# CliffKai/BridgeLang

Hardware: AMD Instinct MI355X
Metric: action-seqs/sec (7-DoF, 224px) openvla-7b bf16 (higher is better)
Workload: dtype bf16; 1 GPU; openvla-7b bf16 inference (BASELINE configs[1]): batch 16 synthetic 224px frames + 32-token prompts per GPU, predict_action = vision towers + projector + Llama prefill S=288 + 6 cached decode steps, greedy; 7 batches in flight: per step one batch is submitted (vision+prefill) while decode iteration g of the batch submitted g steps earlier, g = 1..6, runs as ONE merged 96-row pass over the weights ; batch_per_gpu=16, prompt_len=32, seq_len=288, replicas=1, hip_graph=True, pipeline_depth=7

## Files before the change

### bridgelang_amd/_lib.py

```python
from __future__ import annotations

import ctypes as C
import os
from pathlib import Path

_HERE = Path(__file__).resolve().parent
LIB_PATH = _HERE / "libbridgelang_hip.so"

BL_OK, BL_E_SHAPE, BL_E_ALIGN, BL_E_LAUNCH, BL_E_ARG = 0, -1, -2, -3, -4
_ERR = {BL_E_SHAPE: "BL_E_SHAPE (unsupported shape)", BL_E_ALIGN: "BL_E_ALIGN (alignment)",
        BL_E_LAUNCH: "BL_E_LAUNCH (HIP launch failed)", BL_E_ARG: "BL_E_ARG (null pointer / bad enum)"}

EPI_NONE, EPI_BIAS, EPI_BIAS_GELU, EPI_BIAS_RES, EPI_RES, EPI_SWIGLU, EPI_F32, EPI_F32_BF16R = range(8)
EPI_SWIGLU_KEEP, EPI_BIAS_GELU_KEEP, EPI_SWIGLU_BWD, EPI_GELU_BWD = range(8, 12)


class GemmDesc(C.Structure):
    _fields_ = [
        ("A", C.c_void_p), ("lda", C.c_int64),
        ("W", C.c_void_p), ("ldw", C.c_int64),
        ("C", C.c_void_p), ("ldc", C.c_int64),
        ("M", C.c_int32), ("N", C.c_int32), ("K", C.c_int32),
        ("epilogue", C.c_int32),
        ("bias", C.c_void_p),
# ... 22 lines not shown
        ("k", C.c_void_p), ("k_bs", C.c_int64), ("k_hs", C.c_int64), ("k_rs", C.c_int64),
        ("v", C.c_void_p), ("v_bs", C.c_int64), ("v_hs", C.c_int64), ("v_rs", C.c_int64),
        ("o", C.c_void_p), ("o_bs", C.c_int64), ("o_hs", C.c_int64), ("o_rs", C.c_int64),
        ("key_mask", C.c_void_p), ("mask_bs", C.c_int64),
        ("B", C.c_int32), ("H", C.c_int32), ("Sq", C.c_int32), ("Skv", C.c_int32), ("head_dim", C.c_int32),
        ("causal", C.c_int32),
        ("scale", C.c_float),
    ]


_vp, _i32, _i64, _u32, _f32 = C.c_void_p, C.c_int32, C.c_int64, C.c_uint32, C.c_float

SIGNATURES = {
    "bl_abi_version": (C.c_int, []),
    "bl_build_arch": (C.c_char_p, []),
    "bl_fill_synth_bf16": (C.c_int, [_vp, _i64, _u32, _f32, _f32, _vp]),
    "bl_fill_synth_bf16_2d": (C.c_int, [_vp, _i64, _i64, _i64, _u32, _f32, _f32, _vp]),
    "bl_pack_weight_bf16": (C.c_int, [_vp, _i64, _i64, _i64, _vp, _vp]),
    "bl_gemm_fp8": (C.c_int, [C.POINTER(GemmDesc), _vp, _vp, _vp]),
    "bl_quantize_rows_fp8": (C.c_int, [_vp, _i64, _i32, _i32, _vp, _i64, _vp, _vp]),
    "bl_colamax_bf16": (C.c_int, [_vp, _i64, _i32, _i32, _vp, _vp]),
    "bl_transpose_quantize_fp8": (C.c_int, [_vp, _i64, _i32, _i32, _vp, _vp, _i64, _i32, _vp, _vp]),
    "bl_gemm_bf16": (C.c_int, [C.POINTER(GemmDesc), _vp]),
    "bl_gemm_skinny_bf16": (C.c_int, [C.POINTER(GemmDesc), _vp]),
    "bl_gemm_skinny_rows_bf16": (C.c_int, [C.POINTER(GemmDesc), _vp]),
    "bl_gemm_tn_bf16": (C.c_int, [C.POINTER(GemmDesc), _vp]),
    "bl_rmsnorm_skinny_bf16": (C.c_int, [_vp, _i64, _vp, _vp, _i64, _i32, _i32, _f32, _vp]),
    "bl_layernorm_bf16": (C.c_int, [_vp, _i64, _vp, _vp, _vp, _i64, _i32, _i32, _f32, _vp]),
    "bl_rmsnorm_bf16": (C.c_int, [_vp, _i64, _vp, _vp, _i64, _i32, _i32, _f32, _vp]),
    "bl_attention_bf16": (C.c_int, [C.POINTER(AttnDesc), _vp]),
    "bl_attention_rope_bf16": (C.c_int, [C.POINTER(AttnDesc), _vp, _vp, _i32, _vp, _vp, _i32, _vp]),
    "bl_attention_lse_bf16": (C.c_int, [C.POINTER(AttnDesc), _vp, _vp]),
    "bl_attention_backward_bf16": (C.c_int, [C.POINTER(AttnDesc), _vp, _vp, _vp, _vp, _vp, _vp, _vp]),
    "bl_attention_decode_bf16": (C.c_int, [C.POINTER(AttnDesc), _vp]),
    "bl_attention_decode_rope_bf16": (C.c_int, [C.POINTER(AttnDesc), _vp, _vp, _i32, _vp]),
    "bl_attention_decode_rope_pos_bf16": (C.c_int, [C.POINTER(AttnDesc), _vp, _vp, _i32, _vp, _vp]),
    "bl_attention_decode_rope_grouped_bf16": (C.c_int, [C.POINTER(AttnDesc), _vp, _vp, _i32, _vp, _vp, _vp, _vp]),
    "bl_rope_kvcache_bf16": (C.c_int, [_vp, _i32, _i32, _i32, _i32, _vp, _vp, _i32, _vp, _vp, _i32, _vp]),
    "bl_embed_splice_bf16": (C.c_int, [_vp, _i32, _i32, _vp, _i32, _i32, _vp, _vp]),
    "bl_argmax_f32": (C.c_int, [_vp, _i64, _i32, _i32, _vp, _vp]),
    "bl_cross_entropy_f32": (C.c_int, [_vp, _i64, _i32, _i32, _vp, _i64, _vp, _vp, _vp]),
    "bl_cross_entropy_backward_f32": (C.c_int, [_vp, _i64, _i32, _i32, _vp, _i64, _vp, _vp, _i64, _vp]),
    "bl_rmsnorm_backward_bf16": (C.c_int, [_vp, _i64, _vp, _vp, _i64, _vp, _i64, _vp, _i64, _vp, _vp, _i64, _i32, _i32, _f32, _vp]),
    "bl_layernorm_backward_bf16": (C.c_int, [_vp, _i64, _vp, _vp, _i64, _vp, _i64, _vp, _i64, _vp, _vp, _vp, _i64, _i32, _i32, _f32, _vp]),
    "bl_colsum_bf16": (C.c_int, [_vp, _i64, _i32, _i32, _vp, _vp, _i64, _vp]),
    "bl_swiglu_bf16": (C.c_int, [_vp, _i64, _vp, _i64, _i64, _i32, _vp]),
# ... 63 lines not shown
```

### bridgelang_amd/csrc/gemm_bf16.hip

```cpp
#include "gemm_common.h"
#include <stdlib.h>

namespace bl_gemm_bf16_impl {
using namespace blgemm;

constexpr int BK = 64;
constexpr int ROW_BYTES = 128;
constexpr int GROUP_M = 4;

__device__ __forceinline__ void lin_to_tile(const GemmArgs& p, int lin, int& tm, int& tn) {
  const int width = GROUP_M * p.tiles_n, grp = lin / width, first = grp * GROUP_M;
  const int gsz = min(p.tiles_m - first, GROUP_M), rem = lin - grp * width;
  tm = first + rem % gsz;
  tn = rem / gsz;
}

__device__ __forceinline__ void tile_coords(const GemmArgs& p, int& tm, int& tn) {
  const int nwg = gridDim.x;
  const int orig = blockIdx.x, xcd = orig & 7, q = nwg >> 3, r = nwg & 7;
  const int lin = (xcd < r ? xcd * (q + 1) : r * (q + 1) + (xcd - r) * q) + (orig >> 3);
  const int width = GROUP_M * p.tiles_n, grp = lin / width, first = grp * GROUP_M;
  const int gsz = min(p.tiles_m - first, GROUP_M), rem = lin - grp * width;
  tm = first + rem % gsz;
  tn = rem / gsz;
// ... 210 lines not shown
    BL_KSTEP(0, 1, kt);
    BL_KSTEP(1, 0, kt + 1);
  }
  if (nk & 1) BL_KSTEP(0, 1, nk - 1);
#undef BL_KSTEP
#undef BL_READ
  asm volatile("s_waitcnt vmcnt(0)" ::: "memory");
#undef BL_PIECE
  if (sliced) {
    float* slab = p.slab + (long)blockIdx.y * p.M * p.N;
#pragma unroll
    for (int i = 0; i < NT; ++i)
#pragma unroll
      for (int j = 0; j < MT; ++j) {
        const int m = m0 + wm * TM + j * 16 + l15, n = n0 + wn * TN + i * 16 + lg * 4;
        if (m < p.M && n < p.N) *(f32x4_t*)(slab + (long)m * p.N + n) = acc[i][j];
      }
    return;
  }
  int ncol[NT];
#pragma unroll
  for (int i = 0; i < NT; ++i) ncol[i] = n0 + wn * TN + i * 16 + lg * 4;
  epilogue_tile<EPI, NT, MT>(p, m0 + wm * TM + l15, ncol, m0 + BM, n0 + BN, acc);
#endif
}

template <int EPI>
__global__ __launch_bounds__(256) void gemm128_splitk_reduce_kernel(GemmArgs p) {
#if defined(__HIP_DEVICE_COMPILE__)
  const int n4 = p.N >> 2;
  const long total = (long)p.M * n4;
  for (long i = (long)blockIdx.x * 256 + threadIdx.x; i < total; i += (long)gridDim.x * 256) {
    const int m = (int)(i / n4), n = (int)(i - (long)m * n4) * 4;
    f32x4_t sum = *(const f32x4_t*)(p.slab + (long)m * p.N + n);
    for (int s2 = 1; s2 < p.splitk; ++s2) sum += *(const f32x4_t*)(p.slab + ((long)s2 * p.M + m) * p.N + n);
    epilogue_store4<EPI>(p, m, n, sum);
  }
#endif
}

template <int EPI>
__global__ __launch_bounds__(256) void gemm_rows_tree_reduce_kernel(GemmArgs p) {
#if defined(__HIP_DEVICE_COMPILE__)
  const int n4 = p.N >> 2, S = p.splitk;
  const long total = (long)p.M * n4, stride = (long)p.M * p.N;
  for (long i = (long)blockIdx.x * 256 + threadIdx.x; i < total; i += (long)gridDim.x * 256) {
// ... 948 lines not shown
        lds_attr(&gemm_ring8_kernel<EPI, 64, 64, 4>, ring8_lds_bytes(64, 64)) &&
        lds_attr(&gemm_mid2_kernel<EPI, 1>, 3 * (160 * ROW_BYTES + 4096)) &&
        lds_attr(&gemm_mid2_kernel<EPI, 4>, 3 * (160 * ROW_BYTES + 4 * 4096)) &&
        lds_attr(&gemm_mid2_kernel<EPI, 2, 2>, 2 * (160 * ROW_BYTES + 2 * 4096)) &&
        mid_attr<EPI, 2, 4>() && mid_attr<EPI, 4, 4>() && mid_attr<EPI, 5, 4>() && mid_attr<EPI, 2, 1>() &&
        mid_attr<EPI, 4, 1>() && mid_attr<EPI, 5, 1>();
    return ok ? BL_OK : BL_E_LAUNCH;
  }();
  return rc;
}

template <int EPI>
void launch_slab_reduce(const GemmArgs& p, hipStream_t s) {
  const long work = (long)p.M * (p.N / 4);
  hipLaunchKernelGGL((gemm128_splitk_reduce_kernel<EPI>), dim3((int)min((work + 255) / 256, 2048L)), dim3(256), 0, s, p);
}

template <int EPI, int MB>
void launch_mid(const GemmArgs& p, hipStream_t s, bool wide, dim3 grid) {
  if (wide) hipLaunchKernelGGL((gemm_mid_kernel<EPI, MB, 4>), grid, dim3(256), (mid_lds_bytes<MB, 4>()), s, p);
  else hipLaunchKernelGGL((gemm_mid_kernel<EPI, MB, 1>), grid, dim3(256), (mid_lds_bytes<MB, 1>()), s, p);
}

template <int EPI>
int launch_gemm(const GemmArgs& a, hipStream_t s) {
  if (set_lds_attr<EPI>() != BL_OK) return BL_E_LAUNCH;
  GemmArgs p = a;
  const int bm = (p.M + 255) / 256, bn = (p.N + 255) / 256, big_tiles = bm * bn;
  const bool big = big_tiles >= 128 && p.K >= 512;
  const bool mid2_only = p.M > 320;
  if (p.M <= 640 && p.M > 32 && p.K >= 512 && !(mid2_only && (p.slab || (p.N % 32)))) {
    const int slabs64 = (p.N + 63) / 64, nkm = p.K / BK;
    bool wide = slabs64 >= 160;
    int S = 1;
    if (!wide && p.slab && slabs64 * 2 <= CUS) {
      int S2 = min(8, CUS / slabs64);
      while (S2 > 1 && (nkm / S2 < 8 || p.slab_bytes < (long)S2 * p.M * p.N * 4)) --S2;
      if (S2 > 1) { wide = true; S = S2; }
    }
    if (S == 1 && p.M > 128 && (p.N % 32) == 0) {
      const int mb = (p.M + 159) / 160;
      if (!wide)
        hipLaunchKernelGGL((gemm_mid2_kernel<EPI, 1>), dim3(p.N / 32, mb), dim3(256), 3 * (160 * ROW_BYTES + 4096), s, p);
      else if (slabs64 >= 400)
        hipLaunchKernelGGL((gemm_mid2_kernel<EPI, 4>), dim3((p.N + 127) / 128, mb), dim3(256), 3 * (160 * ROW_BYTES + 4 * 4096), s, p);
      else
        hipLaunchKernelGGL((gemm_mid2_kernel<EPI, 2, 2>), dim3((p.N + 63) / 64, mb), dim3(256), 2 * (160 * ROW_BYTES + 2 * 4096), s, p);
      BL_CHECK_LAUNCH();
      return BL_OK;
    }
    const int slabs = wide ? slabs64 : (p.N + 15) / 16;
    if (S == 1 && !wide && p.slab && slabs < CUS) {
      S = min(8, (CUS + CUS / 2 + slabs - 1) / slabs);
      while (S > 1 && (nkm / S < 8 || p.slab_bytes < (long)S * p.M * p.N * 4)) --S;
    }
    p.splitk = S;
    const dim3 grid(slabs, S);
    if (p.M <= 128) launch_mid<EPI, 2>(p, s, wide, grid);
    else if (p.M <= 256) launch_mid<EPI, 4>(p, s, wide, grid);
    else launch_mid<EPI, 5>(p, s, wide, grid);
    if (S > 1) launch_slab_reduce<EPI>(p, s);
    BL_CHECK_LAUNCH();
    return BL_OK;
  }
  if (!big && p.K >= 512) {
    const int t160 = ((p.M + 159) / 160) * ((p.N + 127) / 128);
    if (t160 <= CUS && t160 >= (3 * CUS) / 4) {
      p.tiles_m = (p.M + 159) / 160;
      p.tiles_n = (p.N + 127) / 128;
      p.tail_base = -1;
      hipLaunchKernelGGL((gemm_ring8_kernel<EPI, 160, 128, 4>), dim3(t160), dim3(512), ring8_lds_bytes(160, 128), s, p);
      BL_CHECK_LAUNCH();
      return BL_OK;
    }
  }
  if (!big) {
    p.tiles_m = (p.M + 127) / 128;
    p.tiles_n = (p.N + 127) / 128;
    const int tiles = p.tiles_m * p.tiles_n, nk128 = p.K / BK;
    int S128 = 1;
    if (p.slab && tiles <= CUS / 2) {
      S128 = min(8, CUS / tiles);
      while (S128 > 1 && (nk128 / S128 < 8 || p.slab_bytes < (long)S128 * p.M * p.N * 4)) --S128;
    }
    if (S128 > 1) {
      p.splitk = S128;
      hipLaunchKernelGGL((gemm_ring8_kernel<EPI, 128, 128, 4>), dim3(tiles, S128), dim3(512), ring8_lds_bytes(128, 128), s, p);
      launch_slab_reduce<EPI>(p, s);
    } else {
      hipLaunchKernelGGL((gemm128_kernel<EPI>), dim3(tiles), dim3(256), LDS128, s, p);
// ... 34 lines not shown
  const bool can_split = tail && S >= 2 && p.K >= 8192 && p.slab && p.slab_bytes >= (long)tail * S * 256 * 256 * 4;
  if (can_split) {
    main_tiles = big_tiles - tail;
    if (main_tiles) launch256(main_tiles);
    p.tail_base = main_tiles;
    p.splitk = S;
    launch256(tail * S);
    hipLaunchKernelGGL((gemm_splitk_reduce_kernel<EPI>), dim3(tail * 32), dim3(512), 0, s, p);
  } else {
    if (tail != 0 && tail <= 64 && main_tiles > tail) main_tiles = big_tiles - tail; else tail = 0;
    launch256(main_tiles);
    if (tail) {
      p.tail_base = main_tiles;
      if (tail <= 16)
        hipLaunchKernelGGL((gemm_ring8_kernel<EPI, 64, 64, 4>), dim3(tail * 16), dim3(512), ring8_lds_bytes(64, 64), s, p);
      else if (tail <= 32)
        hipLaunchKernelGGL((gemm_ring8_kernel<EPI, 128, 64, 4>), dim3(tail * 8), dim3(512), ring8_lds_bytes(128, 64), s, p);
      else
        hipLaunchKernelGGL((gemm_ring8_kernel<EPI, 128, 128, 4>), dim3(tail * 4), dim3(512), ring8_lds_bytes(128, 128), s, p);
    }
  }
  BL_CHECK_LAUNCH();
  return BL_OK;
}

int launch_gemm_tn(const GemmArgs& a, hipStream_t s) {
  static const int attr_rc = lds_attr(&gemm256s_kernel<BL_EPI_F32, true>, LDS256) ? BL_OK : BL_E_LAUNCH;
  if (attr_rc != BL_OK) return attr_rc;
  GemmArgs p = a;
  p.tiles_m = (p.M + 255) / 256;
  p.tiles_n = (p.N + 255) / 256;
  const int tiles = p.tiles_m * p.tiles_n, nk = (p.K + BK - 1) / BK;
  int tail = tiles > CUS ? tiles % CUS : (2 * tiles <= CUS ? tiles : 0);
  int S = tail ? CUS / tail : 1;
  if (tiles <= CUS && S > 8) S = 8;
  if (S > 16) S = 16;
  while (S > 1 && nk / S < 4) --S;
  const bool can_split = tail && S >= 2 && (nk >= 128 || tiles <= CUS) && p.slab &&
                         p.slab_bytes >= (long)tail * S * 256 * 256 * 4;
  const bool persist_ok = (nk % 2) == 0 && ((long)(p.K - 1) * p.lda + p.M) * 2 < (1L << 32) &&
                          ((long)(p.K - 1) * p.ldw + p.N) * 2 < (1L << 32);
  auto launch_main = [&](int grid) {
    if (persist_ok && grid > CUS) {
      GemmArgs pp = p;
      pp.ptiles = grid;
      hipLaunchKernelGGL((gemm256s_kernel<BL_EPI_F32, true>), dim3(CUS), dim3(512), LDS256, s, pp);
// ... 20 lines not shown
extern "C" int bl_gemm_bf16(const bl_gemm_desc* d, void* stream) {
  GemmArgs a;
  const int rc = fill_gemm_args(d, a);
  if (rc != BL_OK) return rc;
  if (d->a_norm_weight) return BL_E_ARG;
  hipStream_t s = (hipStream_t)stream;
  switch (d->epilogue) {
    case BL_EPI_NONE: return launch_gemm<BL_EPI_NONE>(a, s);
    case BL_EPI_BIAS: return launch_gemm<BL_EPI_BIAS>(a, s);
    case BL_EPI_BIAS_GELU: return launch_gemm<BL_EPI_BIAS_GELU>(a, s);
    case BL_EPI_BIAS_RES: return launch_gemm<BL_EPI_BIAS_RES>(a, s);
    case BL_EPI_RES: return launch_gemm<BL_EPI_RES>(a, s);
    case BL_EPI_SWIGLU: return launch_gemm<BL_EPI_SWIGLU>(a, s);
    case BL_EPI_F32: return launch_gemm<BL_EPI_F32>(a, s);
    case BL_EPI_F32_BF16R: return launch_gemm<BL_EPI_F32_BF16R>(a, s);
    case BL_EPI_SWIGLU_KEEP: return launch_gemm<BL_EPI_SWIGLU_KEEP>(a, s);
    case BL_EPI_BIAS_GELU_KEEP: return launch_gemm<BL_EPI_BIAS_GELU_KEEP>(a, s);
    case BL_EPI_SWIGLU_BWD: return launch_gemm<BL_EPI_SWIGLU_BWD>(a, s);
    case BL_EPI_GELU_BWD: return launch_gemm<BL_EPI_GELU_BWD>(a, s);
    default: return BL_E_ARG;
  }
}

extern "C" int bl_gemm_skinny_rows_bf16(const bl_gemm_desc* d, void* stream) {
  GemmArgs a;
  const int rc = fill_gemm_args(d, a);
  if (rc != BL_OK) return rc;
  if (d->M > 128 || (d->K % 256) || d->a_norm_weight) return BL_E_SHAPE;
  if (d->out_group) return BL_E_ARG;
  hipStream_t s = (hipStream_t)stream;
  switch (d->epilogue) {
    case BL_EPI_NONE: return launch_rows_sk<BL_EPI_NONE>(a, s);
    case BL_EPI_RES: return launch_rows_sk<BL_EPI_RES>(a, s);
    case BL_EPI_SWIGLU: return launch_rows_sk<BL_EPI_SWIGLU>(a, s);
    case BL_EPI_F32: return launch_rows_sk<BL_EPI_F32>(a, s);
    case BL_EPI_F32_BF16R: return launch_rows_sk<BL_EPI_F32_BF16R>(a, s);
    default: return BL_E_ARG;
  }
}

extern "C" int bl_gemm_tn_bf16(const bl_gemm_desc* d, void* stream) {
  if (!d || !d->A || !d->W || !d->C) return BL_E_ARG;
  if (d->epilogue != BL_EPI_F32 || d->out_group || d->a_norm_weight) return BL_E_ARG;
  if (d->M <= 0 || d->N <= 0 || d->K <= 0 || (d->M % 8) || (d->N % 8)) return BL_E_SHAPE;
  if ((d->lda % 8) || (d->ldw % 8) || (d->ldc % 4) || d->lda < d->M || d->ldw < d->N || d->ldc < d->N) return BL_E_ALIGN;
  if (!bl_aligned16(d->A) || !bl_aligned16(d->W) || (((uintptr_t)d->C) & 15)) return BL_E_ALIGN;
// ... 10 lines not shown
```

### bridgelang_amd/engine.py

```python
from __future__ import annotations

from typing import List, Optional

import torch

from . import ops
from .ops import EPI_BIAS, EPI_BIAS_GELU, EPI_BIAS_RES, EPI_F32_BF16R, EPI_NONE, EPI_RES, EPI_SWIGLU, Op
from .weights import TowerW, VLAWeights


def rope_tables(head_dim: int, max_pos: int, theta: float, device) -> tuple:
    inv = 1.0 / (theta ** (torch.arange(0, head_dim, 2, dtype=torch.int64).float() / head_dim))
    fr = torch.arange(max_pos, dtype=torch.float32)[:, None] * inv[None, :]
    return fr.cos().to(torch.bfloat16).to(device), fr.sin().to(torch.bfloat16).to(device)


def _fp8_layers(weights: VLAWeights) -> list:
    cache = weights.__dict__.get("_fp8_layers")
    if cache is None:
        cache = [{n: ops.quantize_weight_fp8(ops.unpack_weight(getattr(lw, n))) for n in ("qkv_w", "o_w", "gu_w", "down_w")}
                 for lw in weights.layers]
        weights.__dict__["_fp8_layers"] = cache
    return cache

# ... 51 lines not shown
            self.qkvd, self.actd = z(B, 3 * D), z(B, I)
        self.cos, self.sin = rope_tables(d.head_dim, d.max_pos, d.rope_theta, dev)
        self.ws = torch.empty(64 << 20, dtype=torch.uint8, device=dev) if splitk else None
        if padded:
            if d.head_dim != 128 or not ops.skinny_supported(B, D, EPI_NONE):
                raise NotImplementedError("padded generation needs head_dim 128 and a batch of at most 16")
            self.cache_mask = torch.ones(B, self.cache_len, dtype=torch.uint8, device=dev)
            self.key_mask = self.cache_mask[:, :S]
            self.last_row = torch.full((B,), S - 1, dtype=torch.int64, device=dev)
            self.rope_pos = torch.zeros(n_new, B, dtype=torch.int32, device=dev)
            self.q_last, self.x_last = z(B, 3 * D), z(B, D)
            self._rows = torch.arange(B, device=dev)
        else:
            self.key_mask = torch.ones(B, S, dtype=torch.uint8, device=dev) if use_mask else None
        self.logits_all = z(B * S, d.vocab, dtype=torch.float32) if all_rows else None
        self.fp8 = fp8
        if fp8:
            if d.llm_dim % 128 or d.llm_inter % 128:
                raise ValueError("fp8 prefill needs llm_dim and llm_inter to be multiples of 128")
            self.w8 = _fp8_layers(weights)
            self.h8, self.act8 = z(B * S, D, dtype=torch.uint8), z(B * S, I, dtype=torch.uint8)
            self.sq = z(B * S, dtype=torch.float32)

        self.dino_ops = [] if text_only else self._plan_tower(weights.dino, 0, self.vbuf[0])
        self.siglip_ops = [] if text_only else self._plan_tower(weights.siglip, d.dino.dim, self.vbuf[1])
        self.vision_ops = self.dino_ops + self.siglip_ops
        self._side = torch.cuda.Stream(device=dev) if dev.type == "cuda" else None
        if vision_only:
            self.projector_ops, self.prefill_ops, self.decode_ops = [], [], []
        else:
            self.projector_ops = [] if text_only else self._plan_projector()
            self.prefill_ops = self._plan_prefill()
            self.decode_ops = [self._plan_decode(t) for t in range(1, n_new)]
        self._graph: Optional[torch.cuda.CUDAGraph] = None

    def _g(self, *args, **kw):
        return ops.gemm(*args, workspace=self.ws, **kw)

    def _plan_tower(self, tw: TowerW, feat_col: int, vb: dict) -> List[Op]:
        t, B = tw.dims, self.B
        T, Dm, Hp, hd = t.tokens, t.dim, t.mlp_pad, t.head_dim
        M = B * T
        x = vb["x"][:M * Dm].view(M, Dm)
        h = vb["h"][:M * Dm].view(M, Dm)
        ao = vb["ao"][:M * Dm].view(M, Dm)
        qkv = vb["qkv"][:M * 3 * Dm].view(M, 3 * Dm)
        mlp = vb["mlp"][:M * Hp].view(M, Hp)
        v_col = vb["col"]
        g = lambda *a, **k: ops.gemm(*a, workspace=vb["ws"], **k)
        plan = [ops.im2col_patch14(self.pixel_values, t.chan0, v_col, run=False)]
        if tw.prefix is not None:
            plan.append(ops.write_prefix_tokens(tw.prefix, x, B, T, run=False))
        plan.append(g(v_col, tw.patch_w, x, EPI_BIAS_RES, bias=tw.patch_b, res=tw.pos, res_row_mod=256,
                             out_map=(256, T, t.n_prefix), algo_nk=(Dm, self.dims.patch_k), run=False))
        st = (T * 3 * Dm, hd, 3 * Dm)
        for i, b in enumerate(tw.blocks):
            plan.append(ops.layernorm(x, b.norm1_w, b.norm1_b, h, self.dims.ln_eps, run=False))
            plan.append(g(h, b.qkv_w, qkv, EPI_BIAS, bias=b.qkv_b, run=False))
            plan.append(ops.attention(qkv, qkv[:, Dm:], qkv[:, 2 * Dm:], ao, B=B, H=t.heads, Sq=T, Skv=T, head_dim=hd,
                                      q_strides=st, k_strides=st, v_strides=st, o_strides=(T * Dm, hd, Dm),
                                      causal=False, run=False))
            plan.append(g(ao, b.proj_w, x, EPI_BIAS_RES, bias=b.proj_b, scale=b.ls1, res=x, run=False))
            plan.append(ops.layernorm(x, b.norm2_w, b.norm2_b, h, self.dims.ln_eps, run=False))
            plan.append(g(h, b.fc1_w, mlp, EPI_BIAS_GELU, bias=b.fc1_b, algo_nk=(t.mlp, Dm), run=False))
            if i + 1 < len(tw.blocks):
                plan.append(g(mlp, b.fc2_w, x, EPI_BIAS_RES, bias=b.fc2_b, scale=b.ls2, res=x, algo_nk=(Dm, t.mlp),
                                     run=False))
            else:
                plan.append(g(mlp, b.fc2_w, self.feats[:, feat_col:feat_col + Dm], EPI_BIAS_RES, bias=b.fc2_b,
                                     scale=b.ls2, res=x, out_map=(T, 256, -t.n_prefix), algo_nk=(Dm, t.mlp), run=False))
        return plan

    def _plan_projector(self) -> List[Op]:
        w, B, S, D = self.w, self.B, self.S, self.dims.llm_dim
        return [self._g(self.feats, w.fc1_w, self.p1, EPI_BIAS_GELU, bias=w.fc1_b, run=False),
                self._g(self.p1, w.fc2_w, self.p2, EPI_BIAS_GELU, bias=w.fc2_b, run=False),
                self._g(self.p2, w.fc3_w, self.x.view(B * S, D), EPI_BIAS, bias=w.fc3_b, out_map=(256, S, 1), run=False)]

    def _plan_prefill(self, b0: int = 0, b1: Optional[int] = None) -> List[Op]:
        d, w, S = self.dims, self.w, self.S
        b1 = self.B if b1 is None else b1
        B = b1 - b0
        D, H, hd = d.llm_dim, d.llm_heads, d.head_dim
        rows = slice(b0 * S, b1 * S)
        x3 = self.x[b0:b1]
        x = x3.view(B * S, D)
        h, qkv, ao, act = self.h[rows], self.qkv[rows], self.ao[rows], self.act[rows]
        xd, hdd, aod, actd = self.xd[b0:b1], self.hd[b0:b1], self.aod[b0:b1], self.actd[b0:b1]
        key_mask = self.key_mask[b0:b1] if self.key_mask is not None else None
        plan = [ops.embed_splice(self.input_ids[b0:b1], w.embed, x3, self.n_patches, run=False)]
        self.layer_ends: List[int] = []
        cs = (H * self.cache_len * hd, self.cache_len * hd, hd)
        last_rows_only = not self.all_rows and d.llm_layers > 1
        for l, lw in enumerate(w.layers):
# ... 96 lines not shown
                plan.append(self._g(self.hd, lw.qkv_w, self.qkvd, EPI_NONE, run=False))
                plan.append(ops.rope_kvcache(self.qkvd, self.cos, self.sin, self.k_cache[l], self.v_cache[l], B=B, S=1,
                                             H=H, head_dim=hd, pos0=pos, run=False))
                plan.append(ops.attention_decode(self.qkvd, self.k_cache[l], self.v_cache[l], self.aod, B=B, H=H,
                                                 Skv=pos + 1, head_dim=hd, q_strides=(3 * D, hd, 3 * D), k_strides=cs,
                                                 v_strides=cs, o_strides=(D, hd, D), run=False))
            plan.append(self._g(self.aod, lw.o_w, self.xd, EPI_RES, res=self.xd, run=False))
            if fused:
                plan.append(self._g(self.xd, lw.gu_w, self.actd, EPI_SWIGLU, a_norm=(lw.ln2, d.rms_eps), run=False))
            else:
                plan.append(ops.rmsnorm(self.xd, lw.ln2, self.hd, d.rms_eps, run=False))
                plan.append(self._g(self.hd, lw.gu_w, self.actd, EPI_SWIGLU, run=False))
            plan.append(self._g(self.actd, lw.down_w, self.xd, EPI_RES, res=self.xd, run=False))
        plan += self._head(self.xd, t)
        return plan

    def all_ops(self) -> List[Op]:
        out = self.vision_ops + self.projector_ops + self.prefill_ops
        for step in self.decode_ops:
            out = out + step
        return out

    def run_vision(self) -> None:
        if self._side is None:
            ops.run_all(self.vision_ops)
            return
        main = torch.cuda.current_stream()
        self._side.wait_stream(main)
        with torch.cuda.stream(self._side):
            ops.run_all(self.siglip_ops)
        ops.run_all(self.dino_ops)
        main.wait_stream(self._side)

    def _run_all_stages(self) -> None:
        self.run_vision()
        ops.run_all(self.projector_ops + self.prefill_ops)
        for step in self.decode_ops:
            ops.run_all(step)

    def run_eager(self) -> None:
        self._run_all_stages()

    def capture(self) -> None:
        self.run_eager()
        torch.cuda.synchronize()
        g = torch.cuda.CUDAGraph()
# ... 47 lines not shown
```

### bridgelang_amd/ops.py

```python
from __future__ import annotations

import functools
import math

import ctypes as C
from typing import Optional, Sequence, Tuple

import torch

from . import _lib
from ._lib import (AttnDesc, GemmDesc, EPI_BIAS, EPI_BIAS_GELU, EPI_BIAS_GELU_KEEP, EPI_BIAS_RES, EPI_F32, EPI_F32_BF16R, EPI_GELU_BWD,
                   EPI_NONE, EPI_SWIGLU_BWD, EPI_SWIGLU_KEEP,
                   EPI_RES, EPI_SWIGLU)

__all__ = ["Op", "gemm", "gemm_fp8", "quantize_rows_fp8", "quantize_weight_fp8", "pack_weight", "unpack_weight", "cross_entropy", "layernorm", "rmsnorm", "rmsnorm_skinny", "skinny_rows_supported", "attention", "attention_rope", "attention_decode", "attention_decode_rope", "attention_decode_rope_grouped", "skinny_supported", "rope_kvcache", "embed_splice",
           "argmax", "im2col_patch14", "preprocess_u8", "resample_coeffs", "resize_bicubic_u8", "resize_u8", "crop_resize_bilinear_u8", "write_prefix_tokens", "fill_synth", "run_all",
           "EPI_NONE", "EPI_BIAS", "EPI_BIAS_GELU", "EPI_BIAS_RES", "EPI_RES", "EPI_SWIGLU", "EPI_F32", "EPI_F32_BF16R",
           "EPI_SWIGLU_KEEP", "EPI_BIAS_GELU_KEEP", "EPI_SWIGLU_BWD", "EPI_GELU_BWD"]


def _stream() -> int:
    return torch.cuda.current_stream().cuda_stream


def _bf16(t: torch.Tensor, what: str) -> torch.Tensor:
    if t.dtype != torch.bfloat16 or not t.is_cuda:
        raise TypeError(f"{what}: expected a CUDA/HIP bfloat16 tensor, got {t.dtype} on {t.device}")
    return t


def _rows(t: torch.Tensor, what: str) -> int:
    if t.dim() != 2 or t.stride(1) != 1:
        raise ValueError(f"{what}: expected a 2-D tensor with contiguous last dim, got shape {tuple(t.shape)} "
                         f"stride {t.stride()}")
    return t.stride(0) if t.shape[0] > 1 else max(t.stride(0), t.shape[1])


class Op:
# ... 109 lines not shown
    if use_skinny is None:
        use_skinny = skinny_supported(M, K, epilogue)
    if a_norm is not None:
        if not use_skinny:
            raise ValueError("gemm: a_norm (fused RMSNorm) needs the skinny kernel (M <= 16 and a supported K)")
        d.a_norm_weight, d.a_norm_eps = _bf16(a_norm[0], "a_norm weight").data_ptr(), float(a_norm[1])
        keep.append(a_norm[0])
    if skinny_rows:
        if not skinny_rows_supported(M, K, epilogue) or a_norm is not None or out_map is not None:
            raise ValueError(f"gemm: skinny_rows needs M <= 128, K in {SKINNY_K}, no a_norm / out_map (M={M}, K={K})")
        name = "bl_gemm_skinny_rows_bf16"
    else:
        name = "bl_gemm_skinny_bf16" if use_skinny else "bl_gemm_bf16"
    fn = getattr(lib, name)
    esz = 4 if epilogue in (EPI_F32, EPI_F32_BF16R) else 2
    op = Op(name, fn, (C.byref(d),), (d, *keep),
            flops=2.0 * M * (algo_nk[0] if algo_nk else N) * (algo_nk[1] if algo_nk else K),
            nbytes=2.0 * (M * K + N * K) + esz * M * n_out)
    if run:
        op.run()
    return op


FP8_MAX = 448.0


def quantize_weight_fp8(w: torch.Tensor) -> Tuple[torch.Tensor, torch.Tensor]:
    N, K = w.shape
    if N % 16 or K % 128:
        raise ValueError("quantize_weight_fp8: N % 16 == 0 and K % 128 == 0")
    wf = w.float()
    amax = wf.abs().amax(dim=1)
    scale = torch.where(amax > 0, amax / FP8_MAX, torch.ones_like(amax))
    q = (wf / scale[:, None]).to(torch.float8_e4m3fn)
    packed = pack_weight(q.view(torch.uint8).view(N, K // 2, 2).view(torch.bfloat16).reshape(N, K // 2).contiguous())
    return packed, scale.contiguous()


def quantize_rows_fp8(x: torch.Tensor, q: Optional[torch.Tensor] = None, scales: Optional[torch.Tensor] = None,
                      run: bool = True):
    lib = _lib.load()
    _bf16(x, "x")
    rows, cols = x.shape
    if q is None:
        q = torch.empty(rows, cols, dtype=torch.uint8, device=x.device)
    if scales is None:
# ... 417 lines not shown
```

### include/bridgelang_hip.h

```cpp
#ifndef BRIDGELANG_HIP_H
#define BRIDGELANG_HIP_H

#include <stdint.h>

#ifdef __cplusplus
extern "C" {
#endif

typedef uint16_t bl_bf16;

#define BL_OK 0
#define BL_E_SHAPE (-1)
#define BL_E_ALIGN (-2)
#define BL_E_LAUNCH (-3)
#define BL_E_ARG (-4)

int bl_abi_version(void);
const char* bl_build_arch(void);

int bl_fill_synth_bf16(bl_bf16* dst, int64_t n, uint32_t seed, float mean, float scale, void* stream);
int bl_fill_synth_bf16_2d(bl_bf16* dst, int64_t rows, int64_t cols, int64_t ld, uint32_t seed, float mean,
                          float scale, void* stream);

int bl_pack_weight_bf16(const bl_bf16* src, int64_t ld, int64_t n, int64_t k, bl_bf16* dst, void* stream);
// ... 13 lines not shown
  BL_EPI_GELU_BWD = 11
};

typedef struct bl_gemm_desc {
  const bl_bf16* A;  int64_t lda;
  const bl_bf16* W;  int64_t ldw;
  void* C;           int64_t ldc;
  int32_t M, N, K;
  int32_t epilogue;
  const bl_bf16* bias;
  const bl_bf16* scale;
  const bl_bf16* res; int64_t ldres;
  int32_t res_row_mod;
  int32_t out_group, out_stride, out_offset;
  const bl_bf16* a_norm_weight;
  float a_norm_eps;
  void* workspace;
  int64_t workspace_bytes;
  bl_bf16* C2;
  int64_t ldc2;
} bl_gemm_desc;

int bl_gemm_bf16(const bl_gemm_desc* d, void* stream);

int bl_gemm_skinny_bf16(const bl_gemm_desc* d, void* stream);

int bl_gemm_skinny_rows_bf16(const bl_gemm_desc* d, void* stream);

int bl_gemm_tn_bf16(const bl_gemm_desc* d, void* stream);

int bl_rmsnorm_skinny_bf16(const bl_bf16* x, int64_t ldx, const bl_bf16* w, bl_bf16* y, int64_t ldy, int32_t rows,
                           int32_t dim, float eps, void* stream);

int bl_gemm_fp8(const bl_gemm_desc* d, const float* scale_a, const float* scale_w, void* stream);
int bl_quantize_rows_fp8(const bl_bf16* x, int64_t ldx, int32_t rows, int32_t cols, uint8_t* q, int64_t ldq, float* scales,
                         void* stream);
int bl_colamax_bf16(const bl_bf16* x, int64_t ldx, int32_t rows, int32_t cols, float* amax, void* stream);
int bl_transpose_quantize_fp8(const bl_bf16* x, int64_t ldx, int32_t rows, int32_t cols, const float* amax, uint8_t* q,
                              int64_t ldq, int32_t packed, float* scales, void* stream);

int bl_layernorm_bf16(const bl_bf16* x, int64_t ldx, const bl_bf16* w, const bl_bf16* b, bl_bf16* y, int64_t ldy,
                      int32_t rows, int32_t dim, float eps, void* stream);
int bl_rmsnorm_bf16(const bl_bf16* x, int64_t ldx, const bl_bf16* w, bl_bf16* y, int64_t ldy, int32_t rows,
                    int32_t dim, float eps, void* stream);

typedef struct bl_attn_desc {
// ... 111 lines not shown
```

Measured before the change: 269.1 action-seqs/s.

## Group paired DINO/SigLIP bias-residual GEMMs into one persistent grouped kernel launch

Adds a two-problem grouped GEMM kernel built on the 160x128 ring-buffer tile. Each block walks a combined tile list across both problems and prefetches the next tile's first K-slices while finishing the current one. The vision plan now interleaves the two towers' ops and merges matching bias-residual GEMM pairs into single grouped launches, which is meant to fill the CUs better than two partial-wave launches. This replaces the previous side-stream overlap of the towers with a single-stream interleaved sequence, so the non-grouped ops lose that concurrency.

```diff
diff --git a/bridgelang_amd/_lib.py b/bridgelang_amd/_lib.py
--- a/bridgelang_amd/_lib.py
+++ b/bridgelang_amd/_lib.py
@@ -68,6 +68,7 @@
     "bl_colamax_bf16": (C.c_int, [_vp, _i64, _i32, _i32, _vp, _vp]),
     "bl_transpose_quantize_fp8": (C.c_int, [_vp, _i64, _i32, _i32, _vp, _vp, _i64, _i32, _vp, _vp]),
     "bl_gemm_bf16": (C.c_int, [C.POINTER(GemmDesc), _vp]),
+    "bl_gemm_bf16_group": (C.c_int, [C.POINTER(GemmDesc), _i32, _vp]),
     "bl_gemm_skinny_bf16": (C.c_int, [C.POINTER(GemmDesc), _vp]),
     "bl_gemm_skinny_rows_bf16": (C.c_int, [C.POINTER(GemmDesc), _vp]),
     "bl_gemm_tn_bf16": (C.c_int, [C.POINTER(GemmDesc), _vp]),
diff --git a/bridgelang_amd/csrc/gemm_bf16.hip b/bridgelang_amd/csrc/gemm_bf16.hip
--- a/bridgelang_amd/csrc/gemm_bf16.hip
+++ b/bridgelang_amd/csrc/gemm_bf16.hip
@@ -256,6 +256,174 @@
 #pragma unroll
   for (int i = 0; i < NT; ++i) ncol[i] = n0 + wn * TN + i * 16 + lg * 4;
   epilogue_tile<EPI, NT, MT>(p, m0 + wm * TM + l15, ncol, m0 + BM, n0 + BN, acc);
+#endif
+}
+
+struct GroupArgs {
+  GemmArgs m[2];
+  int tiles0, total;
+};
+
+template <int EPI>
+__global__ __launch_bounds__(512) void gemm_ring8_group_kernel(GroupArgs g) {
+#if defined(__HIP_DEVICE_COMPILE__)
+  constexpr int BM = 160, BN = 128, NST = 4;
+  constexpr int NWAVE = 8, TM = BM / 2, TN = BN / 4, MT = TM / 16, NT = TN / 16;
+  constexpr int APIECES = BM / 8, WPIECES = BN / 8;
+  constexpr int APW = (APIECES + NWAVE - 1) / NWAVE, WPW = WPIECES / NWAVE, LPS = APW + WPW;
+  constexpr int A_BYTES = BM * ROW_BYTES, BUF_BYTES = A_BYTES + BN * ROW_BYTES, DUMP = NST * BUF_BYTES;
+  extern __shared__ __attribute__((aligned(16))) char smem[];
+
+  const int tid = threadIdx.x, lane = tid & 63;
+  const int wave = __builtin_amdgcn_readfirstlane(tid >> 6);
+  const int wm = wave >> 2, wn = wave & 3;
+  const int prow = lane >> 3, pchunk = (lane & 7) ^ prow;
+  const int l15 = lane & 15, lg = lane >> 4;
+  const int c0 = lg ^ (lane & 7);
+  const int offA = (wm * TM + l15) * ROW_BYTES;
+  const int offW = A_BYTES + (wn * NT) * 2048 + lane * 16;
+
+  int mic = 0, min_ = 0;
+  int m0 = 0, n0 = 0, nk = 0, m0n = 0, n0n = 0, nkn = 0;
+  const uint16_t* Ac = nullptr; const uint16_t* Wc = nullptr; const uint16_t* An = nullptr; const uint16_t* Wn = nullptr;
+  unsigned abc = 0u, wbc = 0u, abn = 0u, wbn = 0u;
+  unsigned voffA[APW], voffW[WPW], voffAn[APW], voffWn[WPW];
+  int ldsA[APW];
+#pragma unroll
+  for (int j = 0; j < APW; ++j) ldsA[j] = (j * NWAVE + wave) < APIECES ? (j * NWAVE + wave) * 1024 : -1;
+#define BL_G_SEL(F) (mi__ ? g.m[1].F : g.m[0].F)
+#define BL_G_NEXT(VB)                                                                                            \
+  do {                                                                                                           \
+    abn = 0u; wbn = 0u;                                                                                          \
+    const int vb__ = (VB);                                                                                       \
+    if (vb__ < g.total) {                                                                                        \
+      const int mi__ = vb__ >= g.tiles0 ? 1 : 0;                                                                 \
+      min_ = mi__;                                                                                               \
+      const int tn__ = BL_G_SEL(tiles_n), K__ = BL_G_SEL(K), M__ = BL_G_SEL(M), N__ = BL_G_SEL(N);               \
+      const long lda__ = BL_G_SEL(lda);                                                                          \
+      const int idx__ = mi__ ? vb__ - g.tiles0 : vb__, cnt__ = mi__ ? g.total - g.tiles0 : g.tiles0;             \
+                   \
+      const int xcd__ = idx__ & 7, q__ = cnt__ >> 3, r__ = cnt__ & 7;                                            \
+      const int lin__ = (xcd__ < r__ ? xcd__ * (q__ + 1) : r__ * (q__ + 1) + (xcd__ - r__) * q__) + (idx__ >> 3); \
+      m0n = (lin__ / tn__) * BM; n0n = (lin__ % tn__) * BN;                                                      \
+      nkn = K__ / BK;                                                                                            \
+      An = BL_G_SEL(A); Wn = BL_G_SEL(W);                                                                        \
+      abn = (unsigned)min((long)M__ * lda__ * 2, 0xffffffffL);                                                   \
+      wbn = (unsigned)min((long)N__ * K__ * 2, 0xffffffffL);                                                     \
+      const int kt32__ = K__ >> 5;                                                                               \
+      _Pragma("unroll") for (int j = 0; j < APW; ++j)                                                            \
+        voffAn[j] = ldsA[j] >= 0 ? (unsigned)(((long)(m0n + (j * NWAVE + wave) * 8 + prow) * lda__) * 2 + pchunk * 16) \
+                                 : 0xfffffff0u;                                                                  \
+      _Pragma("unroll") for (int j = 0; j < WPW; ++j) {                                                          \
+        const int blk__ = j * NWAVE + wave;                                                                      \
+        voffWn[j] = (unsigned)(((long)(n0n / 16 + (blk__ >> 1)) * kt32__ + (blk__ & 1)) * 1024 + lane * 16);     \
+      }                                                                                                          \
+    }                                                                                                            \
+  } while (0)
+#define BL_G_ADVANCE()                                                                                           \
+  do {                                                                                                           \
+    mic = min_; m0 = m0n; n0 = n0n; nk = nkn; Ac = An; Wc = Wn; abc = abn; wbc = wbn;                               \
+    _Pragma("unroll") for (int j = 0; j < APW; ++j) voffA[j] = voffAn[j];                                        \
+    _Pragma("unroll") for (int j = 0; j < WPW; ++j) voffW[j] = voffWn[j];                                        \
+  } while (0)
+#define BL_RS(PTR, BYTES) __builtin_amdgcn_make_buffer_rsrc((void*)(PTR), 0, (BYTES), 0x00020000)
+#define BL_PIECE(BUF, T, PC)                                                                                      \
+  do {                                                                                                            \
+    char* base__ = smem + (BUF) * BUF_BYTES;                                                                      \
+    const bool nx__ = (T) >= nk;                                                                                  \
+    const int tt__ = nx__ ? (T) - nk : (T);                                                                       \
+    if ((PC) < APW) {                                                                                             \
+      const int ja__ = (PC) < APW ? (PC) : 0;                                                                     \
+      const __amdgpu_buffer_rsrc_t rs__ = BL_RS(nx__ ? An : Ac, nx__ ? abn : abc);                                \
+      BL_GLDS(rs__, ldsA[ja__] >= 0 ? base__ + ldsA[ja__] : smem + DUMP, nx__ ? voffAn[ja__] : voffA[ja__], tt__ * 128); \
+    } else {                                                                                                      \
+      const int jw__ = (PC) >= APW ? (PC) - APW : 0;                                                              \
+      const __amdgpu_buffer_rsrc_t rs__ = BL_RS(nx__ ? Wn : Wc, nx__ ? wbn : wbc);                                \
+      BL_GLDS(rs__, base__ + A_BYTES + (jw__ * NWAVE + wave) * 1024, nx__ ? voffWn[jw__] : voffW[jw__], tt__ * 2048); \
+    }                                                                                                             \
+  } while (0)
+
+  int vb = blockIdx.x;
+  BL_G_NEXT(vb);
+  BL_G_ADVANCE();
+  BL_G_NEXT(vb + (int)gridDim.x);
+
+  f32x4_t acc[NT][MT];
+#pragma unroll
+  for (int i = 0; i < NT; ++i)
+#pragma unroll
+    for (int j = 0; j < MT; ++j) acc[i][j] = (f32x4_t){0.f, 0.f, 0.f, 0.f};
+
+#pragma unroll
+  for (int s2 = 0; s2 < NST - 1; ++s2) {
+#pragma unroll
+    for (int pc2 = 0; pc2 < LPS; ++pc2) BL_PIECE(s2, s2, pc2);
+  }
+  static_assert((NST - 2) * LPS <= 63 && NST >= 4, "counted vmcnt range / ring depth");
+  constexpr int NMF = 2 * NT * MT, EVERY = NMF / LPS;
+  constexpr int NRD = 2 * (NT + MT), RPG = (NRD + LPS - 1) / LPS;
+  static_assert(EVERY >= 1, "more DMA pieces than MFMAs");
+  bf16x8_t wf[2][2][NT], af[2][2][MT];
+#define BL_READ(SET, BASE, RI)                                                                                   \
+  do {                                                                                                           \
+    const int ks__ = (RI) / (NT + MT), e__ = (RI) % (NT + MT);                                                   \
+    if (e__ < NT) wf[SET][ks__][e__ < NT ? e__ : 0] = *(const bf16x8_t*)((BASE) + offW + e__ * 2048 + ks__ * 1024);   \
+    else af[SET][ks__][e__ >= NT ? e__ - NT : 0] =                                                               \
+        *(const bf16x8_t*)((BASE) + offA + (e__ - NT) * 16 * ROW_BYTES + ((c0 ^ (ks__ * 4)) << 4));              \
+  } while (0)
+#define BL_KSTEP(CUR, NXT, KT)                                                                                   \
+  do {                                                                                                           \
+    asm volatile("s_waitcnt vmcnt(%0)" ::"n"((NST - 3) * LPS) : "memory");    \
+    __builtin_amdgcn_s_barrier();    \
+    const char* nb__ = smem + ((sb + (KT) + 1) % NST) * BUF_BYTES;                                               \
+    const int nslot__ = (sb + (KT) + NST - 1) % NST;                                \
+    const int nkt__ = (KT) + NST - 1;                                                                            \
+    _Pragma("unroll") for (int gq = 0; gq < LPS; ++gq) {                                                         \
+      BL_PIECE(nslot__, nkt__, gq);                                                                              \
+      _Pragma("unroll") for (int ri = gq * RPG; ri < ((gq + 1) * RPG < NRD ? (gq + 1) * RPG : NRD); ++ri)        \
+          BL_READ(NXT, nb__, ri);                                                                                \
+      __builtin_amdgcn_sched_barrier(0);                                                                         \
+      _Pragma("unroll") for (int idx = gq * EVERY; idx < ((gq + 1 < LPS) ? (gq + 1) * EVERY : NMF); ++idx) {     \
+        const int ks = idx / (NT * MT), i = (idx / MT) % NT, j = idx % MT;                                       \
+        acc[i][j] = __builtin_amdgcn_mfma_f32_16x16x32_bf16(wf[CUR][ks][i], af[CUR][ks][j], acc[i][j], 0, 0, 0); \
+      }                                                                                                          \
+      __builtin_amdgcn_sched_barrier(0);                                                                         \
+    }                                                                                                            \
+  } while (0)
+  int sb = 0;
+  asm volatile("s_waitcnt vmcnt(%0)" ::"n"((NST - 2) * LPS) : "memory");
+  __builtin_amdgcn_s_barrier();
+#pragma unroll
+  for (int ri = 0; ri < NRD; ++ri) BL_READ(0, smem, ri);
+  for (;;) {
+    for (int kt = 0; kt < nk; kt += 2) {
+      BL_KSTEP(0, 1, kt);
+      BL_KSTEP(1, 0, kt + 1);
+    }
+    const bool more = abn != 0u;
+    if (!more) asm volatile("s_waitcnt vmcnt(0)" ::: "memory");
+    int ncol[NT];
+#pragma unroll
+    for (int i = 0; i < NT; ++i) ncol[i] = n0 + wn * TN + i * 16 + lg * 4;
+    if (mic == 0) epilogue_tile<EPI, NT, MT>(g.m[0], m0 + wm * TM + l15, ncol, m0 + BM, n0 + BN, acc);
+    else epilogue_tile<EPI, NT, MT>(g.m[1], m0 + wm * TM + l15, ncol, m0 + BM, n0 + BN, acc);
+    if (!more) break;
+    sb = (sb + nk) % NST;
+    vb += (int)gridDim.x;
+    BL_G_ADVANCE();
+    BL_G_NEXT(vb + (int)gridDim.x);
+#pragma unroll
+    for (int i = 0; i < NT; ++i)
+#pragma unroll
+      for (int j = 0; j < MT; ++j) acc[i][j] = (f32x4_t){0.f, 0.f, 0.f, 0.f};
+  }
+#undef BL_KSTEP
+#undef BL_READ
+#undef BL_PIECE
+#undef BL_RS
+#undef BL_G_ADVANCE
+#undef BL_G_NEXT
+#undef BL_G_SEL
 #endif
 }
 
@@ -1250,6 +1418,13 @@
   else hipLaunchKernelGGL((gemm_mid_kernel<EPI, MB, 1>), grid, dim3(256), (mid_lds_bytes<MB, 1>()), s, p);
 }
 
+inline bool one_round_160(const GemmArgs& p) {
+  const bool mid = p.M <= 640 && p.M > 32 && p.K >= 512 && !(p.M > 320 && (p.slab || (p.N % 32)));
+  const bool big = ((p.M + 255) / 256) * ((p.N + 255) / 256) >= 128 && p.K >= 512;
+  const int t160 = ((p.M + 159) / 160) * ((p.N + 127) / 128);
+  return !mid && !big && p.K >= 512 && t160 <= CUS && t160 >= (3 * CUS) / 4;
+}
+
 template <int EPI>
 int launch_gemm(const GemmArgs& a, hipStream_t s) {
   if (set_lds_attr<EPI>() != BL_OK) return BL_E_LAUNCH;
@@ -1291,9 +1466,9 @@
     BL_CHECK_LAUNCH();
     return BL_OK;
   }
-  if (!big && p.K >= 512) {
+  {
     const int t160 = ((p.M + 159) / 160) * ((p.N + 127) / 128);
-    if (t160 <= CUS && t160 >= (3 * CUS) / 4) {
+    if (one_round_160(p)) {
       p.tiles_m = (p.M + 159) / 160;
       p.tiles_n = (p.N + 127) / 128;
       p.tail_base = -1;
@@ -1374,6 +1549,34 @@
   }
   BL_CHECK_LAUNCH();
   return BL_OK;
+}
+
+template <int EPI>
+bool launch_group_160(const GemmArgs& a0, const GemmArgs& a1, hipStream_t s, int& rc) {
+  auto fits = [](const GemmArgs& p) {
+    const int nk = p.K / BK;
+    return one_round_160(p) && (nk % 2) == 0 && nk >= 4 && (long)(p.M + 160) * p.lda * 2 < (1L << 31) &&
+           (long)p.N * p.K * 2 < (1L << 31);
+  };
+  if (!fits(a0) || !fits(a1)) return false;
+  static const int attr_rc =
+      lds_attr(&gemm_ring8_group_kernel<EPI>, ring8_lds_bytes(160, 128)) ? BL_OK : BL_E_LAUNCH;
+  rc = attr_rc;
+  if (rc != BL_OK) return true;
+  GroupArgs g;
+  const bool swap = a1.K > a0.K;
+  g.m[0] = swap ? a1 : a0;
+  g.m[1] = swap ? a0 : a1;
+  for (GemmArgs& p : g.m) {
+    p.tiles_m = (p.M + 159) / 160;
+    p.tiles_n = (p.N + 127) / 128;
+    p.tail_base = -1;
+  }
+  g.tiles0 = g.m[0].tiles_m * g.m[0].tiles_n;
+  g.total = g.tiles0 + g.m[1].tiles_m * g.m[1].tiles_n;
+  hipLaunchKernelGGL((gemm_ring8_group_kernel<EPI>), dim3(min(g.total, CUS)), dim3(512), ring8_lds_bytes(160, 128), s, g);
+  rc = hipGetLastError() == hipSuccess ? BL_OK : BL_E_LAUNCH;
+  return true;
 }
 
 int launch_gemm_tn(const GemmArgs& a, hipStream_t s) {
@@ -1440,6 +1643,26 @@
   }
 }
 
+extern "C" int bl_gemm_bf16_group(const bl_gemm_desc* d, int n, void* stream) {
+  if (!d || n < 1 || n > 2) return BL_E_ARG;
+  if (n == 2) {
+    if (d[0].epilogue != d[1].epilogue) return BL_E_ARG;
+    GemmArgs a[2];
+    for (int i = 0; i < 2; ++i) {
+      const int rc = fill_gemm_args(&d[i], a[i]);
+      if (rc != BL_OK) return rc;
+      if (d[i].a_norm_weight) return BL_E_ARG;
+    }
+    int rc = BL_OK;
+    if (d[0].epilogue == BL_EPI_BIAS_RES && launch_group_160<BL_EPI_BIAS_RES>(a[0], a[1], (hipStream_t)stream, rc)) return rc;
+  }
+  for (int i = 0; i < n; ++i) {
+    const int rc = bl_gemm_bf16(&d[i], stream);
+    if (rc != BL_OK) return rc;
+  }
+  return BL_OK;
+}
+
 extern "C" int bl_gemm_skinny_rows_bf16(const bl_gemm_desc* d, void* stream) {
   GemmArgs a;
   const int rc = fill_gemm_args(d, a);
diff --git a/bridgelang_amd/engine.py b/bridgelang_amd/engine.py
--- a/bridgelang_amd/engine.py
+++ b/bridgelang_amd/engine.py
@@ -97,10 +97,14 @@
             self.h8, self.act8 = z(B * S, D, dtype=torch.uint8), z(B * S, I, dtype=torch.uint8)
             self.sq = z(B * S, dtype=torch.float32)
 
+        self._tower_gemm_calls: dict = {}
         self.dino_ops = [] if text_only else self._plan_tower(weights.dino, 0, self.vbuf[0])
         self.siglip_ops = [] if text_only else self._plan_tower(weights.siglip, d.dino.dim, self.vbuf[1])
         self.vision_ops = self.dino_ops + self.siglip_ops
+        self.vision_group_ops = self._plan_towers_grouped()
+        del self._tower_gemm_calls
         self._side = torch.cuda.Stream(device=dev) if dev.type == "cuda" else None
+        self.group_vision = True
         if vision_only:
             self.projector_ops, self.prefill_ops, self.decode_ops = [], [], []
         else:
@@ -122,7 +126,12 @@
         qkv = vb["qkv"][:M * 3 * Dm].view(M, 3 * Dm)
         mlp = vb["mlp"][:M * Hp].view(M, Hp)
         v_col = vb["col"]
-        g = lambda *a, **k: ops.gemm(*a, workspace=vb["ws"], **k)
+        def g(A, W, out, epi, **k):
+            k.pop("run")
+            call = dict(A=A, W=W, out=out, epilogue=epi, workspace=vb["ws"], **k)
+            op = ops.gemm(**call, run=False)
+            self._tower_gemm_calls[id(op)] = call
+            return op
         plan = [ops.im2col_patch14(self.pixel_values, t.chan0, v_col, run=False)]
         if tw.prefix is not None:
             plan.append(ops.write_prefix_tokens(tw.prefix, x, B, T, run=False))
@@ -145,6 +154,20 @@
                 plan.append(g(mlp, b.fc2_w, self.feats[:, feat_col:feat_col + Dm], EPI_BIAS_RES, bias=b.fc2_b,
                                      scale=b.ls2, res=x, out_map=(T, 256, -t.n_prefix), algo_nk=(Dm, t.mlp), run=False))
         return plan
+
+    def _plan_towers_grouped(self) -> List[Op]:
+        calls = self._tower_gemm_calls
+        a = [op for op in self.dino_ops if op.name != "bl_write_prefix_tokens_bf16"]
+        b = [op for op in self.siglip_ops if op.name != "bl_write_prefix_tokens_bf16"]
+        plan = [op for op in self.dino_ops + self.siglip_ops if op.name == "bl_write_prefix_tokens_bf16"]
+        n = min(len(a), len(b))
+        for x, y in zip(a[:n], b[:n]):
+            cx, cy = calls.get(id(x)), calls.get(id(y))
+            if cx is not None and cy is not None and cx["epilogue"] == cy["epilogue"] == EPI_BIAS_RES:
+                plan.append(ops.gemm_group([cx, cy], run=False))
+            else:
+                plan += [x, y]
+        return plan + a[n:] + b[n:]
 
     def _plan_projector(self) -> List[Op]:
         w, B, S, D = self.w, self.B, self.S, self.dims.llm_dim
@@ -287,6 +310,9 @@
         return out
 
     def run_vision(self) -> None:
+        if self.group_vision:
+            ops.run_all(self.vision_group_ops)
+            return
         if self._side is None:
             ops.run_all(self.vision_ops)
             return
diff --git a/bridgelang_amd/ops.py b/bridgelang_amd/ops.py
--- a/bridgelang_amd/ops.py
+++ b/bridgelang_amd/ops.py
@@ -13,7 +13,7 @@
                    EPI_NONE, EPI_SWIGLU_BWD, EPI_SWIGLU_KEEP,
                    EPI_RES, EPI_SWIGLU)
 
-__all__ = ["Op", "gemm", "gemm_fp8", "quantize_rows_fp8", "quantize_weight_fp8", "pack_weight", "unpack_weight", "cross_entropy", "layernorm", "rmsnorm", "rmsnorm_skinny", "skinny_rows_supported", "attention", "attention_rope", "attention_decode", "attention_decode_rope", "attention_decode_rope_grouped", "skinny_supported", "rope_kvcache", "embed_splice",
+__all__ = ["Op", "gemm", "gemm_group", "gemm_fp8", "quantize_rows_fp8", "quantize_weight_fp8", "pack_weight", "unpack_weight", "cross_entropy", "layernorm", "rmsnorm", "rmsnorm_skinny", "skinny_rows_supported", "attention", "attention_rope", "attention_decode", "attention_decode_rope", "attention_decode_rope_grouped", "skinny_supported", "rope_kvcache", "embed_splice",
            "argmax", "im2col_patch14", "preprocess_u8", "resample_coeffs", "resize_bicubic_u8", "resize_u8", "crop_resize_bilinear_u8", "write_prefix_tokens", "fill_synth", "run_all",
            "EPI_NONE", "EPI_BIAS", "EPI_BIAS_GELU", "EPI_BIAS_RES", "EPI_RES", "EPI_SWIGLU", "EPI_F32", "EPI_F32_BF16R",
            "EPI_SWIGLU_KEEP", "EPI_BIAS_GELU_KEEP", "EPI_SWIGLU_BWD", "EPI_GELU_BWD"]
@@ -169,6 +169,25 @@
     return op
 
 
+def gemm_group(calls: Sequence[dict], run: bool = True) -> Op:
+    lib = _lib.load()
+    if not 1 <= len(calls) <= 2:
+        raise ValueError("gemm_group: one or two member problems")
+    subs = [gemm(**c, run=False) for c in calls]
+    if any(s.name != "bl_gemm_bf16" for s in subs):
+        raise ValueError("gemm_group: members must be tiled-kernel problems (no skinny forms)")
+    descs = (GemmDesc * len(subs))()
+    for i, s in enumerate(subs):
+        C.memmove(C.byref(descs[i]), C.byref(s.keep[0]), C.sizeof(GemmDesc))
+    if len({d.epilogue for d in descs}) != 1:
+        raise ValueError("gemm_group: members must share the epilogue kind")
+    op = Op("bl_gemm_bf16", lib.bl_gemm_bf16_group, (descs, len(subs)), (descs, *[k for s in subs for k in s.keep]),
+            flops=sum(s.flops for s in subs), nbytes=sum(s.bytes for s in subs))
+    if run:
+        op.run()
+    return op
+
+
 FP8_MAX = 448.0
 
 
diff --git a/include/bridgelang_hip.h b/include/bridgelang_hip.h
--- a/include/bridgelang_hip.h
+++ b/include/bridgelang_hip.h
@@ -59,6 +59,8 @@
 } bl_gemm_desc;
 
 int bl_gemm_bf16(const bl_gemm_desc* d, void* stream);
+
+int bl_gemm_bf16_group(const bl_gemm_desc* d, int n, void* stream);
 
 int bl_gemm_skinny_bf16(const bl_gemm_desc* d, void* stream);
 
```

New measurement: 266.9 action-seqs/s. About the same (-0.8%).
